# JINXER000/GIE-mapping

Measured on AMD Instinct MI355X. Metric: edt_map_update_throughput, higher is better.
Workload: dtype int32; 1 GPU; 512x512x512 @ 0.05 m, sensor-less hash world (BASELINE config 5): occupied iff hash(x,y,z) < 1 %, full observation, 25 ~; preset=c5, fast_mode=False, tiles=single volume, blocks=360448

## Files before the change

gie-mapping_amd/csrc/gie_api.inc.h:

```cpp
#include <stdio.h>
#include <stdlib.h>
#include <string.h>
#include <math.h>
#include <string>
#include <vector>

#include <cstdio>
#include <unistd.h>
static const char *const gie_kernel_names[GIE_K_NUM] = { "ogm_classify", "ray_register", "ray_free", "ray_finalize", "block_alloc", "fuse",
       "edt_pass_y", "edt_pass_x", "edt_pass_z", "mark", "frontiers", "wave_a", "wave_b", "waves", "commit", "edt_prep", "mark_commit",
       "ground_frontier", "ground_nf1", "ground", "ground_query", "cloud", "los", "los_query", "sdf", "sdf_query" };

#define GIE_REHASH_PERIOD 64
static thread_local std::string g_gie_err;
static void gie_set_err(const std::string &s) { g_gie_err = s; }
extern "C" const char *gie_last_error(void) { return g_gie_err.c_str(); }

enum gie_owed {
    GIE_OWED_NONE,
    GIE_OWED_FRESH,
    GIE_OWED_STALE
};
struct gie_pivots { int pvt[3], upvt[3], tb0[3]; };
struct gie_pair_state {
// ... 1237 lines not shown
    const int n = (face < 0 || face > 5) ? -1 : gie_face_count(m->c, face);
    if (n < 0 || count < 0 || count > n || (count > 0 && !in)) { gie_set_err("gie_halo_import_sparse: bad arguments"); return GIE_ERR_INVALID; }
    if (count == 0) return GIE_OK;
    char *d = (char *)gie_scratch(m, 1, (size_t)count * sizeof(gie_halo_entry) + 16, "gie_halo_import_sparse");
    if (!d) return GIE_ERR_DEVICE;
    be_h2d(&m->be, d, &count, sizeof(int32_t));
    be_h2d(&m->be, d + 16, in, (size_t)count * sizeof(gie_halo_entry));
    rc = gie_halo_import_sparse_dev(m, face, (const gie_halo_entry *)(d + 16), (const int32_t *)d);
    be_sync(&m->be);
    return rc;
}
static int gie_face_set_of(const gie_ctx &c, const void *const p[6], gie_face_set *fs)
{
    int n = 0;
    for (int f = 0; f < 6; f++) { fs->off[f] = n; if (p[f]) n += gie_face_count(c, f); }
    fs->off[6] = n;
    return n;
}
extern "C" int gie_halo_export_all_dev(gie_mapper *m, gie_halo_voxel *const d_out[6])
{
    int rc = gie_need_pose(m, "gie_halo_export_all"); if (rc) return rc;
    if (!d_out) { gie_set_err("gie_halo_export_all: bad arguments"); return GIE_ERR_INVALID; }
    gie_table_for_pose(m);
    op_halo_export_all op;
    const int n = gie_face_set_of(m->c, (const void *const *)d_out, &op.fs);
    for (int f = 0; f < 6; f++) op.out[f] = d_out[f];
    be_lin(&m->be, m->c, op, n);
    return GIE_OK;
}
extern "C" int gie_halo_import_all_dev(gie_mapper *m, const gie_halo_voxel *const d_in[6])
{
    int rc = gie_need_pose(m, "gie_halo_import_all"); if (rc) return rc;
    if (!d_in) { gie_set_err("gie_halo_import_all: bad arguments"); return GIE_ERR_INVALID; }
    op_halo_need_all nd; op_halo_import_all im;
    const int n = gie_face_set_of(m->c, (const void *const *)d_in, &nd.fs);
    im.fs = nd.fs;
    for (int f = 0; f < 6; f++) { nd.in[f] = d_in[f]; im.in[f] = d_in[f]; }
    if (n == 0) return GIE_OK;
    be_lin(&m->be, m->c, nd, n);
    gie_ghost_block_alloc(m);
    be_lin(&m->be, m->c, im, n);
    return GIE_OK;
}
extern "C" int gie_refine(gie_mapper *m, int32_t *seeded)
{
    int rc = gie_need_pose(m, "gie_refine"); if (rc) return rc;
    gie_table_for_pose(m);
    gie_ctx &c = m->c;
    {
        gie_clear_list l; l.n = 0;
        l.p[l.n] = c.cnt + GIE_CNT_C; l.bytes[l.n++] = sizeof(int32_t);
        l.p[l.n] = c.cnt + GIE_CNT_BAR_B; l.bytes[l.n++] = 2 * sizeof(int32_t);
        l.p[l.n] = c.lvl_next; l.bytes[l.n++] = 2 * GIE_MAX_LEVELS * sizeof(int32_t);
        be_clear(&m->be, l, c.gate);
    }
    const int nb = 2 * (c.X * c.Y + c.Y * c.Z + c.X * c.Z);
    be_lin(&m->be, c, op_refine(), nb);
    gie_pp_set_fused(m);
    be_waves(&m->be, c, 0, 0, 0);
    if (!c.fused) be_vox_list<true>(&m->be, c, op_commit(), c.tl_known, GIE_CNT_TL_KNOWN, 0);
    if (!seeded) return GIE_OK;
    rc = gie_sync(m);
    *seeded = m->h_cnt[GIE_CNT_FRONT_C];
    return rc;
}
extern "C" int gie_round_gate(gie_mapper *m, const int32_t *d_go)
{
    if (!m) { gie_set_err("gie_round_gate: null handle"); return GIE_ERR_INVALID; }
    m->c.gate = d_go;
    return GIE_OK;
}
extern "C" int gie_refine_dev(gie_mapper *m, int32_t *d_changed)
{
    if (!d_changed) { gie_set_err("gie_refine_dev: bad arguments"); return GIE_ERR_INVALID; }
    int rc = gie_refine(m, nullptr); if (rc) return rc;
    be_round_note(&m->be, m->c, d_changed, m->d_round_stats, nullptr, 0);
    return GIE_OK;
}
extern "C" int gie_round_end(gie_mapper *m, const int32_t *d_go)
{
    if (!m) { gie_set_err("gie_round_end: null handle"); return GIE_ERR_INVALID; }
    m->c.gate = nullptr;
    be_round_note(&m->be, m->c, nullptr, m->d_round_stats, d_go, 1);
    return GIE_OK;
}
extern "C" int gie_round_stats(gie_mapper *m, int64_t out[4])
{
    if (!m || !out) { gie_set_err("gie_round_stats: bad arguments"); return GIE_ERR_INVALID; }
    long long v[4] = { 0, 0, 0, 0 };
    be_d2h(&m->be, v, m->d_round_stats, sizeof(v));
    for (int i = 0; i < 4; i++) out[i] = (int64_t)v[i];
    return gie_sync(m);
}
extern "C" int gie_get_stream(gie_mapper *m, void **stream)
{
    if (!m || !stream) { gie_set_err("gie_get_stream: bad arguments"); return GIE_ERR_INVALID; }
    *stream = be_stream_handle(&m->be);
    return GIE_OK;
}

#if defined(GIE_TEST_HOOKS)
extern "C" int gie_debug_place_probe(gie_mapper *m, int reps, float *ms)
{
    if (!m || !ms || m->has_pose) { gie_set_err("gie_debug_place_probe: only on a fresh mapper"); return GIE_ERR_INVALID; }
    *ms = be_place_probe(&m->be, m->c, reps > 0 ? (reps & 0xffff) : 3, (reps >> 16) ? (reps >> 16) : 15);
    return gie_sync(m);
}
extern "C" int gie_debug_fault_barrier(gie_mapper *m, int updates)
{
    if (!m || updates < 0) { gie_set_err("gie_debug_fault_barrier: bad arguments"); return GIE_ERR_INVALID; }
    m->bar_fault_left = updates;
    return GIE_OK;
}
extern "C" int gie_debug_nbr_check(gie_mapper *m, int32_t *mismatches)
{
    if (!m || !mismatches) { gie_set_err("gie_debug_nbr_check: bad arguments"); return GIE_ERR_INVALID; }
    int32_t *d = (int32_t *)gie_scratch(m, 0, sizeof(int32_t), "gie_debug_nbr_check");
    if (!d) return GIE_ERR_DEVICE;
    be_memset(&m->be, d, 0, sizeof(int32_t));
    op_nbr_check op; op.bad = d;
    be_lin(&m->be, m->c, op, 6 * m->c.max_blocks);
    be_d2h(&m->be, mismatches, d, sizeof(int32_t));
    return gie_sync(m);
}
enum { GIE_DBG_TS_PREV_VALID = 0, GIE_DBG_TS_COC_DEFER, GIE_DBG_TS_LAZY_OK, GIE_DBG_TS_ZSTREAM, GIE_DBG_TS_ZWIDE, GIE_DBG_TS_ZFAIL,
       GIE_DBG_TS_LAZY_EXACT, GIE_DBG_TS_TSKIP, GIE_DBG_TS_STATE1, GIE_DBG_TS_STATE2, GIE_DBG_TS_NUM };
extern "C" int gie_debug_tile_state(gie_mapper *m, uint8_t *tknown, uint8_t *tskip, uint8_t *tlazy, int32_t *tmax, int32_t *tbmax,
                                    uint32_t *zredo, int32_t *scalars)
{
    if (!m || !scalars) { gie_set_err("gie_debug_tile_state: bad arguments"); return GIE_ERR_INVALID; }
    const gie_ctx &c = m->c;
    const size_t ntile = (size_t)c.tfd[0] * c.tfd[1] * c.tfd[2];
    if (be_sync(&m->be) != 0) return GIE_ERR_DEVICE;
    if (tknown) be_d2h(&m->be, tknown, c.tknown, ntile);
    if (tskip) be_d2h(&m->be, tskip, c.tskip, ntile);
    if (tlazy) be_d2h(&m->be, tlazy, c.tlazy, ntile);
    if (tmax) be_d2h(&m->be, tmax, c.tmax, ntile * sizeof(int32_t));
    if (tbmax) be_d2h(&m->be, tbmax, c.tbmax, ntile * sizeof(int32_t));
    if (zredo) be_d2h(&m->be, zredo, c.zredo, (size_t)((c.X + 15) / 16) * c.Y * sizeof(uint32_t));
    int32_t cnt[GIE_CNT_NUM];
    be_d2h(&m->be, cnt, c.cnt, sizeof(cnt));
    scalars[GIE_DBG_TS_PREV_VALID] = m->pp.owed == GIE_OWED_FRESH;
    scalars[GIE_DBG_TS_COC_DEFER] = c.coc_defer;
    scalars[GIE_DBG_TS_LAZY_OK] = c.lazy_ok;
    scalars[GIE_DBG_TS_ZSTREAM] = cnt[GIE_CNT_ZSTREAM];
    scalars[GIE_DBG_TS_ZWIDE] = cnt[GIE_CNT_ZWIDE];
    scalars[GIE_DBG_TS_ZFAIL] = cnt[GIE_CNT_ZFAIL];
    scalars[GIE_DBG_TS_LAZY_EXACT] = cnt[GIE_CNT_LAZY_EXACT];
    scalars[GIE_DBG_TS_TSKIP] = cnt[GIE_CNT_TSKIP];
    scalars[GIE_DBG_TS_STATE1] = cnt[GIE_CNT_STATE1];
    scalars[GIE_DBG_TS_STATE2] = cnt[GIE_CNT_STATE2];
    return be_sync(&m->be) != 0 ? GIE_ERR_DEVICE : GIE_OK;
}
extern "C" int gie_debug_set_frame(gie_mapper *m, int ct)
{
    if (!m || ct < 0) { gie_set_err("gie_debug_set_frame: bad arguments"); return GIE_ERR_INVALID; }
    if (m->merge_open) { gie_set_err("gie_debug_set_frame: a merge is open (gie_merge_end first)"); return GIE_ERR_INVALID; }
    m->c.map_ct = ct;
    return GIE_OK;
}
#endif
extern "C" int gie_profile_enable(gie_mapper *m, int on)
{
    if (!m) { gie_set_err("gie_profile_enable: null handle"); return GIE_ERR_INVALID; }
    be_prof_enable(&m->be, on);
    return GIE_OK;
}
extern "C" int gie_profile_read(gie_mapper *m, gie_kernel_time *out, int max_entries)
{
    if (!m || !out || max_entries < GIE_K_NUM) { gie_set_err("gie_profile_read: need room for all kernels"); return GIE_ERR_INVALID; }
    float ms[GIE_K_NUM]; int n[GIE_K_NUM];
    be_prof_collect(&m->be, ms, n, GIE_K_NUM);
    int k = 0;
    for (int i = 0; i < GIE_K_NUM; i++) {
        if (i == GIE_K_GROUND_FRONTIER && !m->gfr.planes) continue;
        memset(out[k].name, 0, sizeof(out[k].name));
        strncpy(out[k].name, gie_kernel_names[i], sizeof(out[k].name) - 1);
        out[k].total_ms = ms[i]; out[k].launches = n[i];
        k++;
    }
    return k;
}
```

gie-mapping_amd/csrc/gie_hip.hip:

```cpp
#include <cstdio>
#include <unistd.h>
#include <cstring>
#include <cstdlib>
#include <string>
#include <algorithm>
#include <vector>
#include <hip/hip_runtime.h>
#include <hip/hip_ext.h>
#include <rocprim/rocprim.hpp>
#include "gie_kernels.hip.h"

#define GIE_NEV 8

struct be_state {
    int device;
    int num_cu;
    int cu_total;
    hipStream_t stream;
    hipEvent_t ev[GIE_NEV];
    int ev_set[GIE_NEV];
    void *scan_tmp; size_t scan_bytes;
    void *arena;
    hipEvent_t copy_ev[2];
    hipStream_t side;
// ... 281 lines not shown
    const size_t tile = ((size_t)c.Z * (TX + 1) + 3) & ~(size_t)3;
    const size_t lds = tile * 4 + (size_t)WAVES * LP * 8 + (size_t)LP * 2 + 16;
    static bool attr_done = false;
    if (!attr_done) {
        GIE_HIP_OK(hipFuncSetAttribute(reinterpret_cast<const void *>(&k_edt_z<CP, TX, WAVES>), hipFuncAttributeMaxDynamicSharedMemorySize, 160 * 1024));
        attr_done = true;
    }
    const int ntx = (c.X + TX - 1) / TX, ntiles = ntx * c.Y;
    int wgs = (int)((160 * 1024) / (lds + 256));
    if (wgs < 1) wgs = 1; if (wgs > 4) wgs = 4;
    int grid = wgs * b->cu_total; if (grid > (ntiles + 1) / 2) grid = (ntiles + 1) / 2;
    GIE_LAUNCH(b, (k_edt_z<CP, TX, WAVES>), dim3(grid), dim3(64 * WAVES), lds, c, ntx, ntiles, full);
}
template <int CP> static void gie_launch_edt_xz(be_state *b, const gie_ctx &c, bool zpass, int full, int zs_fused = 0, bool redo = false)
{
    if (redo) {
        GIE_LAUNCH(b, k_edt_x_redo<CP>, dim3(b->cu_total * 8), dim3(64 * GIE_EDTX_WAVES), 0, c);
    } else if (!zpass) {
        GIE_LAUNCH(b, k_edt_x<CP>, dim3((c.Y + GIE_EDTX_WAVES - 1) / GIE_EDTX_WAVES, c.Z), dim3(64 * GIE_EDTX_WAVES), 0, c, zs_fused, full);
    } else {
        gie_launch_edt_z<CP, 16, 8>(b, c, full);
    }
}
static void gie_launch_edt_dim(be_state *b, const gie_ctx &c, int L, bool zpass, int full, int zs_fused = 0, bool redo = false)
{
    if (L <= 64) gie_launch_edt_xz<1>(b, c, zpass, full, zs_fused, redo);
    else if (L <= 128) gie_launch_edt_xz<2>(b, c, zpass, full, zs_fused, redo);
    else if (L <= 256) gie_launch_edt_xz<4>(b, c, zpass, full, zs_fused, redo);
    else if (L <= 512) gie_launch_edt_xz<8>(b, c, zpass, full, zs_fused, redo);
    else gie_launch_edt_xz<16>(b, c, zpass, full, zs_fused, redo);
}
static int be_zs_mode(const gie_ctx &c)
{
    if (c.Z < 64 || c.Z > 1024) return 0;
    static const int fused = GIE_SWITCH("GIE_ZS_FUSED", 1);
    return (fused && (c.X & 1) == 0) ? 2 : 1;
}
static int be_edt_z_stream(be_state *b, const gie_ctx &c, int full);
static void be_edt_z_rest(be_state *b, const gie_ctx &c, int full, int zs)
{
    if (zs == 2) gie_launch_edt_dim(b, c, c.X, false, full, 0, true);
    gie_launch_edt_dim(b, c, c.Z, true, full);
}
static void be_edt_z(be_state *b, const gie_ctx &c, int full) { be_edt_z_rest(b, c, full, be_edt_z_stream(b, c, full) ? be_zs_mode(c) : 0); }
#define GIE_VOXA_MULT 32
template <bool STAGED, class F> static void be_vox_list(be_state *b, const gie_ctx &c, const F &f, const int32_t *list, int count_idx, int always_list)
{
    GIE_LAUNCH(b, (k_voxa<F, STAGED>), dim3(b->cu_total * GIE_VOXA_MULT), dim3(256), 0, c, f, list, count_idx, always_list);
}
#define GIE_MARKC_MULT 64
#define GIE_MARKC_LAZY_MULT 40
static void be_markc(be_state *b, const gie_ctx &c, const int32_t *list)
{
    const dim3 g(b->cu_total * ((c.coc_defer && c.lazy_ok) ? GIE_MARKC_LAZY_MULT : GIE_MARKC_MULT)), t(256);
    GIE_LAUNCH(b, k_markc, g, t, 0, c, list);
}
static float be_place_probe(be_state *b, const gie_ctx &c, int reps, int streams = 15)
{
    const long long ntile = (long long)c.tfd[0] * c.tfd[1] * c.tfd[2];
    const int nslot = (int)(ntile < c.max_blocks ? ntile : c.max_blocks);
    hipEvent_t e0, e1;
    if (hipEventCreate(&e0) != hipSuccess || hipEventCreate(&e1) != hipSuccess) return -1.f;
    std::vector<float> ms;
    hipLaunchKernelGGL(k_place_probe, dim3(b->cu_total * GIE_MARKC_MULT), dim3(256), 0, b->stream, c, nslot, streams);
    for (int r = 0; r < reps; r++) {
        (void)hipEventRecord(e0, b->stream);
        hipLaunchKernelGGL(k_place_probe, dim3(b->cu_total * GIE_MARKC_MULT), dim3(256), 0, b->stream, c, nslot, streams);
        (void)hipEventRecord(e1, b->stream);
        (void)hipEventSynchronize(e1);
        float t = 0.f; (void)hipEventElapsedTime(&t, e0, e1); ms.push_back(t);
    }
    (void)hipEventDestroy(e0); (void)hipEventDestroy(e1);
    std::sort(ms.begin(), ms.end());
    GIE_HIP_OK(hipMemsetAsync(c.pair, 0, (size_t)c.N * sizeof(uint64_t), b->stream));
    return ms.empty() ? -1.f : ms[ms.size() / 2];
}
#define GIE_ROWS_MULT 32
static void be_fuse(be_state *b, const gie_ctx &c, const int32_t *list)
{
    if (c.pntcld_mode) GIE_LAUNCH(b, k_fuse_rows<true>, dim3(b->cu_total * GIE_ROWS_MULT), dim3(256), 0, c, op_fuse(), list);
    else GIE_LAUNCH(b, k_fuse_rows<false>, dim3(b->cu_total * GIE_ROWS_MULT), dim3(256), 0, c, op_fuse(), list);
}
static void be_frontier_tiles(be_state *b, const gie_ctx &c, const int32_t *known, int known_idx, const int32_t *list, int count_idx)
{
    gie_face_patches fp;
    const int da[6] = { c.Y, c.Y, c.X, c.X, c.X, c.X }, db[6] = { c.Z, c.Z, c.Z, c.Z, c.Y, c.Y };
    fp.off[0] = 0;
    for (int f = 0; f < 6; f++) { fp.na[f] = (da[f] + 7) / 8; fp.off[f + 1] = fp.off[f] + fp.na[f] * ((db[f] + 7) / 8); }
    const long long ntile = (long long)c.tfd[0] * c.tfd[1] * c.tfd[2];
    int nsum = (int)((ntile + 64 * GIE_FF_WAVES - 1) / (64 * GIE_FF_WAVES));
    if (nsum > 2 * b->cu_total) nsum = 2 * b->cu_total;
    const int nface = (fp.off[6] + GIE_FF_WAVES - 1) / GIE_FF_WAVES;
    GIE_LAUNCH(b, k_frontier_faces, dim3(nsum + nface), dim3(64 * GIE_FF_WAVES), 0, c, fp, known, known_idx, nsum);
    static int mult = 0;
    if (mult <= 0) {
        if (hipOccupancyMaxActiveBlocksPerMultiprocessor(&mult, reinterpret_cast<const void *>(&k_frontier_tiles), 64 * GIE_FR_WAVES, 0) != hipSuccess || mult < 1) mult = 2;
    }
    GIE_LAUNCH(b, k_frontier_tiles, dim3(b->cu_total * mult), dim3(64 * GIE_FR_WAVES), 0, c, list, count_idx);
}
static void be_edt_z_direct(be_state *b, const gie_ctx &c)
{
    GIE_LAUNCH(b, k_edt_z_direct, dim3(b->cu_total * 16), dim3(256), 0, c);
}
#define GIE_ZSTREAM_WAVES 8
static int be_edt_z_stream(be_state *b, const gie_ctx &c, int full)
{
    const int zs = be_zs_mode(c);
    if (!zs) return 0;
    const int nxr = (c.X + 63) / 64;
    const long long want = (long long)b->cu_total * 4 * GIE_ZSTREAM_WAVES;
    int nseg = (int)((want + (long long)nxr * c.Y - 1) / ((long long)nxr * c.Y));
    const int maxseg = c.Z / 64 > 0 ? c.Z / 64 : 1;
    if (nseg > maxseg) nseg = maxseg; if (nseg < 1) nseg = 1;
    int seg_len = ((c.Z + nseg - 1) / nseg + 31) & ~31;
    nseg = (c.Z + seg_len - 1) / seg_len;
    const long long waves = (long long)nxr * nseg * c.Y;
    long long grid = (waves + 3) / 4;
    const long long cap = (long long)b->cu_total * 8 * 4;
    if (grid > cap) grid = cap;
    if (!full && grid < (long long)b->cu_total * 16) grid = (long long)b->cu_total * 16;
    if (zs == 2) GIE_LAUNCH(b, k_edt_z_stream<true>, dim3((unsigned)grid), dim3(256), 0, c, full, nseg, seg_len, zs);
    else GIE_LAUNCH(b, k_edt_z_stream<false>, dim3((unsigned)grid), dim3(256), 0, c, full, nseg, seg_len, zs);
    return 1;
}
static void be_tile_oldskip(be_state *b, const gie_ctx &c, const int pupvt[3])
{
    const int ntile = c.tfd[0] * c.tfd[1] * c.tfd[2];
    int32_t *const count = &c.cnt[GIE_CNT_STATE1];
    GIE_LAUNCH(b, k_tile_oldskip, dim3((ntile + 255) / 256), dim3(256), 0, c, ntile, c.wc_list[0], count);
    if (c.catchup_fast) GIE_LAUNCH(b, k_coc_catchup_new, dim3(b->cu_total * 8), dim3(256), 0, c, pupvt[0], pupvt[1], pupvt[2], c.wc_list[0], count);
}
static void be_pair_materialise(be_state *b, const gie_ctx &c, int stay)
{
    const int ntile = c.tfd[0] * c.tfd[1] * c.tfd[2];
    int32_t *const count = &c.cnt[GIE_CNT_STATE2];
    GIE_LAUNCH(b, k_pair_lazy_list, dim3((ntile + 255) / 256), dim3(256), 0, c, ntile, stay, c.wc_list[1], count);
    GIE_LAUNCH(b, k_pair_lazy_run, dim3(b->cu_total * 8), dim3(256), 0, c, c.wc_list[1], count);
}
static void be_coc_catchup(be_state *b, const gie_ctx &c, const gie_catchup &p)
{
    const int ntile = c.tfd[0] * c.tfd[1] * c.tfd[2];
    int32_t *const count = &c.cnt[GIE_CNT_STATE1];
    GIE_HIP_OK(hipMemsetAsync(count, 0, sizeof(int32_t), b->stream));
    GIE_LAUNCH(b, k_coc_catchup_list, dim3((ntile + 255) / 256), dim3(256), 0, c, p, ntile, c.wc_list[0], count);
    GIE_LAUNCH(b, k_coc_catchup_run, dim3(b->cu_total * 4), dim3(256), 0, c, p, c.wc_list[0], count);
}
static void be_edt_prep(be_state *b, const gie_ctx &c)
{
    const int ncol = c.tfd[0] * c.tfd[1];
    GIE_LAUNCH(b, k_edt_prep, dim3((ncol + GIE_PREP_WAVES - 1) / GIE_PREP_WAVES), dim3(64 * GIE_PREP_WAVES), 0, c, ncol);
}
static void be_edt(be_state *b, const gie_ctx &c, int full)
{
    dim3 gy((c.X + GIE_EDTY_COLS - 1) / GIE_EDTY_COLS, c.Z);
    be_prof(b, GIE_K_EDT_Y, 0);
    if ((c.X & 3) == 0) {
        const int yb = c.Y > 512 ? 32 : 16, nq = (c.Y + yb - 1) / yb;
        dim3 g4((c.X / 4 + GIE_EDTY4_LANES - 1) / GIE_EDTY4_LANES, c.Z), b4(GIE_EDTY4_LANES, nq);
        if (yb == 16) GIE_LAUNCH(b, k_edt_y4<16>, g4, b4, 0, c);
        else GIE_LAUNCH(b, k_edt_y4<32>, g4, b4, 0, c);
    }
    else if (c.Y <= 256) GIE_LAUNCH(b, (k_edt_y<8, 8>), gy, dim3(GIE_EDTY_COLS, 8), 0, c);
    else if (c.Y <= 512) GIE_LAUNCH(b, (k_edt_y<16, 16>), gy, dim3(GIE_EDTY_COLS, 16), 0, c);
    else GIE_LAUNCH(b, (k_edt_y<32, 16>), gy, dim3(GIE_EDTY_COLS, 16), 0, c);
    be_prof(b, GIE_K_EDT_Y, 1);
    const int zs = be_zs_mode(c);
    be_prof(b, GIE_K_EDT_X, 0); gie_launch_edt_dim(b, c, c.X, false, full, zs == 2 ? zs : 0); be_prof(b, GIE_K_EDT_X, 1);
    be_prof(b, GIE_K_EDT_Z, 0);
    const int zl = be_edt_z_stream(b, c, full);
    if (!zl && !full) be_edt_z_direct(b, c);
    be_edt_z_rest(b, c, full, zl ? zs : 0);
    be_prof(b, GIE_K_EDT_Z, 1);
}
template <class F> static void be_chained(be_state *b, const F &enqueue)
{
    std::lock_guard<std::mutex> lock(g_waves_mutex);
    const int dv = b->device & 63;
    (void)hipSetDevice(b->device);
    const bool chain = g_live_mappers[dv] > 1;
    if (chain) {
        if (g_waves_event_set[dv]) GIE_HIP_OK(hipStreamWaitEvent(b->stream, g_waves_event[dv], 0));
        else { GIE_HIP_OK(hipEventCreateWithFlags(&g_waves_event[dv], hipEventDisableTiming)); g_waves_event_set[dv] = true; }
    }
    enqueue();
    if (chain) GIE_HIP_OK(hipEventRecord(g_waves_event[dv], b->stream));
}
static void be_waves(be_state *b, const gie_ctx &c, int with_ab, int record_seeds, int clear_first)
{
    be_chained(b, [&]() {
        if (clear_first) {
            GIE_HIP_OK(hipMemsetAsync(&c.cnt[GIE_CNT_BAR_B], 0, 2 * sizeof(int32_t), b->stream));
            GIE_HIP_OK(hipMemsetAsync(c.lvl_next, 0, 2 * GIE_MAX_LEVELS * sizeof(int32_t), b->stream));
        }
        if (with_ab) GIE_LAUNCH(b, k_waves_ab, dim3(b->num_cu), dim3(GIE_WAVE_THREADS), 0, c);
        GIE_LAUNCH(b, k_waves_c, dim3(b->num_cu), dim3(GIE_WAVE_THREADS), 0, c, with_ab, record_seeds);
    });
}

#include "gie_api.inc.h"
#include "gie_sdf.inc.h"
#include "gie_nf1.inc.h"
#include "gie_costmat.inc.h"
#include "gie_frontier.inc.h"
#include "gie_los.inc.h"
#include "gie_path.inc.h"
#include "gie_cloud.inc.h"
#include "gie_ground.inc.h"
#include "gie_ground_nf1.inc.h"
#include "gie_ground_los.inc.h"
#include "gie_ground_frontier.inc.h"
#include "gie_ground_costmat.inc.h"
#include "gie_ground_view.inc.h"
#include "gie_ground_rollout.inc.h"
#include "gie_ground_footprint.inc.h"
#include "gie_ground_pose_nf1.inc.h"
```

gie-mapping_amd/csrc/gie_kernels.hip.h:

```cpp
#ifndef GIE_KERNELS_HIP_H
#define GIE_KERNELS_HIP_H

#include <hip/hip_runtime.h>
#include "gie_functors.h"

#if defined(GIE_WAVE_TIMING) || defined(GIE_RAY_TIMING)
#include "../../tools/measure/gie_timing.h"
#endif
#if !defined(GIE_WAVE_TIMING)
#define GIE_TS2(tag, n) do { } while (0)
#define GIE_WPROF_DECL do { } while (0)
#define GIE_WPROF_MARK(base) do { } while (0)
#define GIE_WPROF_ADD(i, v) do { } while (0)
#define GIE_WPROF_END(base) do { } while (0)
#define GIE_WPROF_DRAIN() do { } while (0)
#define GIE_WPROF_SUB(i) do { } while (0)
#define GIE_WPROF_SUBSTART() do { } while (0)
#define GIE_WPROF_DUMP() do { } while (0)
#define GIE_WPROF_CLK() 0ull
#define GIE_WAVE_TIMING_RESET(cond) do { } while (0)
#endif
#if !defined(GIE_RAY_TIMING)
#define GIE_RTS(k) do { } while (0)
#endif
// ... 179 lines not shown
    if (walk) {
        int stop = 0x7fffffff;
        bool more = true;
        for (int k0 = 0; k0 < max_steps && more && stop == 0x7fffffff; k0 += GIE_RAY_BATCH) {
            if (*(volatile int *)&s_stop[lane] < base) break;
            int ids[GIE_RAY_BATCH], end[GIE_RAY_BATCH];
            bool went[GIE_RAY_BATCH];
#pragma unroll
            for (int j = 0; j < GIE_RAY_BATCH; j++) {
                went[j] = gie_dda_before(d, Tn);
                end[j] = 0; ids[j] = -1;
                if (went[j]) { int lx, ly, lz; end[j] = gie_dda_step(d); ids[j] = gie_ray_cell(c, d, lx, ly, lz); }
            }
            int8_t ty[GIE_RAY_BATCH];
#pragma unroll
            for (int j = 0; j < GIE_RAY_BATCH; j++) ty[j] = ids[j] >= 0 ? c.inst_type[ids[j]] : (int8_t)GIE_VOX_UNKNOWN;
#pragma unroll
            for (int j = 0; j < GIE_RAY_BATCH; j++) {
                if (stop != 0x7fffffff || !went[j]) continue;
                if (ty[j] == GIE_VOX_OCCUPIED) stop = base + k0 + j;
                else if (end[j]) stop = base + k0 + j + 1;
            }
            more = went[GIE_RAY_BATCH - 1];
        }
        if (stop != 0x7fffffff) atomicMin(&s_stop[lane], stop);
    }
    GIE_RTS(2);
    __syncthreads();
    GIE_RTS(3);
    const int stop = s_stop[lane];
    d = at_start;
    for (int k = 0; k < max_steps; k++) {
        int id = -1;
        const bool went = walk && base + k < stop && gie_dda_before(d, Tn);
        if (went) {
            int lx, ly, lz;
            gie_dda_step(d);
            id = gie_ray_cell(c, d, lx, ly, lz);
            if (id >= 0) gie_ray_touch_k(c, d, lx, ly, lz, &last_tile);
        }
        if (__ballot(went) == 0ull) break;
        if (__ballot(id >= 0) == 0ull) continue;
        gie_wave_add(c, id, -1);
    }
    GIE_RTS(4);
}

__device__ __forceinline__ void gie_clear_part(const gie_clear_list &l, int w)
{
    int r = 0, nw = gie_clear_wgs(l.bytes[0]);
    while (w >= nw && r + 1 < l.n) { w -= nw; r++; nw = gie_clear_wgs(l.bytes[r]); }
    if (w >= nw) return;
    unsigned char *p = (unsigned char *)l.p[r];
    const uint32_t bytes = l.bytes[r];
    const uint32_t head = (uint32_t)((16u - ((uintptr_t)p & 15u)) & 15u) < bytes ? (uint32_t)((16u - ((uintptr_t)p & 15u)) & 15u) : bytes;
    const uint32_t nvec = (bytes - head) / 16u, tail0 = head + nvec * 16u;
    const uint32_t tid = (uint32_t)w * 256u + threadIdx.x, nth = (uint32_t)nw * 256u;
    for (uint32_t i = tid; i < head; i += nth) p[i] = 0;
    uint4 *v = (uint4 *)(p + head);
    for (uint32_t i = tid; i < nvec; i += nth) v[i] = make_uint4(0, 0, 0, 0);
    for (uint32_t i = tail0 + tid; i < bytes; i += nth) p[i] = 0;
}
__global__ __launch_bounds__(256) void k_clear(const gie_clear_list l, const int32_t *gate)
{
    if (gate != nullptr && *(const volatile int32_t *)gate == 0) return;
    gie_clear_part(l, (int)blockIdx.x);
}

__global__ __launch_bounds__(256) void k_flush_clear(const gie_ctx c, const op_pair_flush f, const int n, const gie_clear_list l, const int nclr)
{
    if ((int)blockIdx.x >= nclr) { const int i = ((int)blockIdx.x - nclr) * 256 + (int)threadIdx.x; if (i < n) f(c, i); return; }
    gie_clear_part(l, (int)blockIdx.x);
}

__global__ __launch_bounds__(256) void k_cell_alloc(const gie_ctx c, const int ncell)
{
    if (GIE_GATE_CLOSED(c)) return;
    const int i = blockIdx.x * 256 + threadIdx.x;
    int found = -1;
    bool isnew = false;
    if (i < ncell) {
        const int bx = i % c.tdim[0], by = (i / c.tdim[0]) % c.tdim[1], bz = i / (c.tdim[0] * c.tdim[1]);
        found = gie_cell_prev_slot(c, bx, by, bz);
        if (found < 0) found = gie_hash_find(c, bx + c.tb0[0], by + c.tb0[1], bz + c.tb0[2]);
        isnew = found < 0 && (c.blk_need[i] || (c.scan_labels && gie_block_observed(c, c.scan_labels, bx, by, bz)));
        c.blk_need[i] = 0;
    }
    __shared__ int s_cnt[4], s_base[4];
    const int lane = __lane_id(), wave = threadIdx.x >> 6;
    const unsigned long long m = __ballot(isnew);
    if (lane == 0) s_cnt[wave] = __popcll(m);
    __syncthreads();
    const int c0 = s_cnt[0], c1 = s_cnt[1], c2 = s_cnt[2], c3 = s_cnt[3];
    const int cnt = c0 + c1 + c2 + c3;
    if (cnt > 0) {
        if (threadIdx.x == 0) {
            int ftop = 0, nf = 0, base = 0;
            if (c.retain > 0) { ftop = atomicSub(&c.pool_count[1], cnt); nf = ftop < 0 ? 0 : (ftop < cnt ? ftop : cnt); }
            if (cnt > nf) base = atomicAdd(&c.pool_count[0], cnt - nf);
            const int lbase = atomicAdd(&c.cnt[GIE_CNT_NEWLIST], cnt);
            atomicAdd(&c.cnt[GIE_CNT_NEWBLK], cnt);
            s_base[0] = base; s_base[1] = lbase; s_base[2] = nf; s_base[3] = ftop;
        }
        __syncthreads();
        if (isnew) {
            const int base = s_base[0], lbase = s_base[1], nf = s_base[2], ftop = s_base[3];
            const int before = (wave > 0 ? c0 : 0) + (wave > 1 ? c1 : 0) + (wave > 2 ? c2 : 0);
            const int r = before + __popcll(m & ((1ull << lane) - 1ull));
            const int slot = gie_alloc_slot(c, r, nf, ftop, base);
            if (slot >= c.max_blocks) { gie_aor32(&c.cnt[GIE_CNT_ERR], GIE_ERRF_POOL); c.blk_new[lbase + r] = -1; }
            else { gie_cell_insert(c, i, slot); c.blk_new[lbase + r] = slot; found = slot; }
        }
    }
    if (i < ncell) {
        c.blk_tab[i] = found;
        if (found >= 0) gie_cell_mark_tiles(c, i);
    }
}
__global__ __launch_bounds__(256) void k_block_init_list(const gie_ctx c, const int ninit, const int ntile)
{
    if (GIE_GATE_CLOSED(c)) return;
    if ((int)blockIdx.x >= ninit) {
        const op_fuse_list f;
        const int nfl = (int)gridDim.x - ninit;
        for (int i0 = ((int)blockIdx.x - ninit) * 256; i0 < ntile; i0 += nfl * 256) {
            const int i = i0 + (int)threadIdx.x;
            f(c, i < ntile ? i : -1);
        }
        return;
    }
    const int n = c.cnt[GIE_CNT_NEWLIST];
    if (blockIdx.x == 0 && threadIdx.x == 0) {
        if (c.pool_count[0] > c.max_blocks) c.pool_count[0] = c.max_blocks;
        if (c.pool_count[1] < 0) c.pool_count[1] = 0;
    }
    for (int e = blockIdx.x; e < n; e += ninit) {
        const int slot = c.blk_new[e];
        if (slot < 0) continue;
        gie_init_voxel(c, slot, threadIdx.x);
        gie_init_voxel(c, slot, threadIdx.x + 256);
        if (threadIdx.x < 6) gie_nbr_link(c, slot, (int)threadIdx.x);
    }
}

#ifndef GIE_EDTY_COLS
#define GIE_EDTY_COLS 64
#endif
template <int YW, int TPC>
__global__ __launch_bounds__(GIE_EDTY_COLS * TPC) void k_edt_y(const gie_ctx c)
{
    constexpr int QW = YW / TPC;
    __shared__ uint32_t s_bits[YW][GIE_EDTY_COLS];
    const int col = threadIdx.x, q = threadIdx.y;
    const int x = blockIdx.x * GIE_EDTY_COLS + col;
    const int z = blockIdx.y;
    if (!c.zocc[z]) return;
    const int X = c.X, Y = c.Y;
    const bool in = x < X;
    const int8_t *t = c.glb_type + (size_t)z * X * Y + (in ? x : 0);
#pragma unroll
    for (int j = 0; j < QW; j++) {
        const int w = q * QW + j;
        uint32_t m = 0;
        if (in && w * 32 < Y) {
#pragma unroll
            for (int k = 0; k < 32; k++) {
                const int y = w * 32 + k;
                if (y < Y) m |= (uint32_t)(t[(size_t)y * X] == GIE_VOX_OCCUPIED) << k;
            }
        }
        s_bits[w][col] = m;
    }
    __syncthreads();
    if (!in) return;
    uint32_t bits[YW];
#pragma unroll
    for (int w = 0; w < YW; w++) bits[w] = s_bits[w][col];
    int prev_last[YW], next_first[YW];
    int last = -1;
#pragma unroll
    for (int w = 0; w < YW; w++) { prev_last[w] = last; if (bits[w]) last = w * 32 + 31 - __clz(bits[w]); }
    int first = -1;
#pragma unroll
    for (int w = YW - 1; w >= 0; w--) { next_first[w] = first; if (bits[w]) first = w * 32 + __ffs(bits[w]) - 1; }
    uint16_t *out = c.cy1 + (size_t)z * X * Y + x;
#pragma unroll
    for (int w = 0; w < YW; w++) {
        if (w / QW != q) continue;
        if (w * 32 >= Y) break;
        const uint32_t bw = bits[w];
        const int pl = prev_last[w], nf = next_first[w];
        for (int k = 0; k < 32; k++) {
            const int y = w * 32 + k;
            if (y >= Y) break;
            const uint32_t lo = bw & (0xffffffffu >> (31 - k));
            const int below = lo ? w * 32 + 31 - __clz(lo) : pl;
            const uint32_t hi = bw >> k;
            const int above = hi ? y + __ffs(hi) - 1 : nf;
            int r;
            if (above >= 0 && (below < 0 || above - y <= y - below)) r = above; else r = below;
            out[(size_t)y * X] = r < 0 ? (uint16_t)0xffff : (uint16_t)r;
        }
    }
}

#define GIE_EDTY4_LANES 16
template <int YB>
__global__ __launch_bounds__(32 * GIE_EDTY4_LANES) void k_edt_y4(const gie_ctx c)
{
    __shared__ __attribute__((aligned(16))) uint32_t s_m[32][GIE_EDTY4_LANES * 4];
    const int l = threadIdx.x, q = threadIdx.y, nq = blockDim.y;
    const int x = (blockIdx.x * GIE_EDTY4_LANES + l) * 4;
    const int z = blockIdx.y;
    if (!c.zocc[z]) return;
    const int X = c.X, Y = c.Y;
    const bool in = x < X;
    const size_t base = (size_t)z * X * Y + (in ? x : 0);
    uint32_t m[4] = {0u, 0u, 0u, 0u};
    if (in) {
        const int8_t *t = c.glb_type + base;
        uint32_t v[YB];
#pragma unroll
        for (int k = 0; k < YB; k++) {
            const int y = q * YB + k;
            v[k] = *reinterpret_cast<const uint32_t *>(t + (size_t)min(y, Y - 1) * X);
        }
        const uint32_t ymask = (q * YB + YB <= Y) ? 0xffffffffu : ((q * YB < Y) ? (0xffffffffu >> (32 - (Y - q * YB))) : 0u);
#pragma unroll
        for (int k = 0; k < YB; k++) {
#pragma unroll
            for (int cc = 0; cc < 4; cc++) m[cc] |= (uint32_t)(((v[k] >> (8 * cc)) & 0xffu) == (uint32_t)GIE_VOX_OCCUPIED) << k;
        }
#pragma unroll
        for (int cc = 0; cc < 4; cc++) m[cc] &= ymask;
    }
    *reinterpret_cast<uint4 *>(&s_m[q][4 * l]) = make_uint4(m[0], m[1], m[2], m[3]);
    __syncthreads();
    if (!in) return;
    int pl[4] = {-1, -1, -1, -1}, nf[4] = {-1, -1, -1, -1};
    for (int w = 0; w < q; w++) {
        const uint4 o = *reinterpret_cast<const uint4 *>(&s_m[w][4 * l]);
        const uint32_t ow[4] = {o.x, o.y, o.z, o.w};
#pragma unroll
        for (int cc = 0; cc < 4; cc++) if (ow[cc]) pl[cc] = w * YB + 31 - __clz(ow[cc]);
    }
    for (int w = nq - 1; w > q; w--) {
        const uint4 o = *reinterpret_cast<const uint4 *>(&s_m[w][4 * l]);
        const uint32_t ow[4] = {o.x, o.y, o.z, o.w};
#pragma unroll
        for (int cc = 0; cc < 4; cc++) if (ow[cc]) nf[cc] = w * YB + __ffs(ow[cc]) - 1;
    }
    uint16_t *out = c.cy1 + base;
#pragma unroll
    for (int k = 0; k < YB; k++) {
        const int y = q * YB + k;
        if (y >= Y) break;
        uint32_t r4[4];
#pragma unroll
        for (int cc = 0; cc < 4; cc++) {
            const uint32_t bw = m[cc];
            const uint32_t lo = bw & (0xffffffffu >> (31 - k));
            const int below = lo ? q * YB + 31 - __clz(lo) : pl[cc];
            const uint32_t hi = bw >> k;
            const int above = hi ? y + __ffs(hi) - 1 : nf[cc];
            int r;
            if (above >= 0 && (below < 0 || above - y <= y - below)) r = above; else r = below;
            r4[cc] = r < 0 ? 0xffffu : (uint32_t)r;
        }
        *reinterpret_cast<uint2 *>(out + (size_t)y * X) = make_uint2(r4[0] | (r4[1] << 16), r4[2] | (r4[3] << 16));
    }
}

__device__ __forceinline__ void gie_wave_sync()
{
    __builtin_amdgcn_fence(__ATOMIC_RELEASE, "wavefront");
    __builtin_amdgcn_wave_barrier();
    __builtin_amdgcn_fence(__ATOMIC_ACQUIRE, "wavefront");
}

__device__ __forceinline__ uint32_t gie_scan_sites(const uint2 *ce, const int up, const int lo, const int hi)
{
    uint32_t b0 = 0xffffffffu, b1 = 0xffffffffu, b2 = 0xffffffffu, b3 = 0xffffffffu;
    for (int j = lo; j <= hi; j += 4) {
        const uint2 v0 = ce[j], v1 = ce[min(j + 1, hi)], v2 = ce[min(j + 2, hi)], v3 = ce[min(j + 3, hi)];
        const int d0 = up - (int)(v0.y & 0xffffu), d1 = up - (int)(v1.y & 0xffffu);
        const int d2 = up - (int)(v2.y & 0xffffu), d3 = up - (int)(v3.y & 0xffffu);
        b0 = min(b0, (uint32_t)__mul24(d0, d0) + v0.x);
        b1 = min(b1, (uint32_t)__mul24(d1, d1) + v1.x);
        b2 = min(b2, (uint32_t)__mul24(d2, d2) + v2.x);
        b3 = min(b3, (uint32_t)__mul24(d3, d3) + v3.x);
    }
    return min(min(b0, b1), min(b2, b3));
}

template <int CP>
__device__ __forceinline__ void gie_row_argmin(const uint2 *ce, const int K, const int L, const int lane, int (&sj)[CP])
{
    const int u0 = lane * CP;
    int s0;
    {
        const int g8 = lane & ~7, r = lane & 7;
        const int ug = g8 * CP;
        uint32_t b0 = 0xffffffffu, b1 = 0xffffffffu, b2 = 0xffffffffu, b3 = 0xffffffffu;
        {
            const int up = ug << 5, kl = K - 1;
            for (int j = r; j < K; j += 32) {
                const uint2 v0 = ce[j], v1 = ce[min(j + 8, kl)], v2 = ce[min(j + 16, kl)], v3 = ce[min(j + 24, kl)];
                const int d0 = up - (int)(v0.y & 0xffffu), d1 = up - (int)(v1.y & 0xffffu);
                const int d2 = up - (int)(v2.y & 0xffffu), d3 = up - (int)(v3.y & 0xffffu);
                b0 = min(b0, (uint32_t)__mul24(d0, d0) + v0.x);
                b1 = min(b1, (uint32_t)__mul24(d1, d1) + v1.x);
                b2 = min(b2, (uint32_t)__mul24(d2, d2) + v2.x);
                b3 = min(b3, (uint32_t)__mul24(d3, d3) + v3.x);
            }
        }
        uint32_t bg = min(min(b0, b1), min(b2, b3));
        bg = min(bg, (uint32_t)__shfl_xor((int)bg, 1));
        bg = min(bg, (uint32_t)__shfl_xor((int)bg, 2));
        bg = min(bg, (uint32_t)__shfl_xor((int)bg, 4));
        const int sg = (ug < L) ? (int)(bg & 1023u) : K - 1;
        int sn = __shfl_down(sg, 8);
        if (lane >= 56) sn = K - 1;
        s0 = sg;
        if (r != 0 && u0 < L && sn > sg) s0 = (int)(gie_scan_sites(ce, u0 << 5, sg, sn) & 1023u);
        if (u0 >= L) s0 = K - 1;
    }
    int sup = __shfl_down(s0, 1);
    if (lane == 63) sup = K - 1;
    int sx[CP + 1];
    sx[0] = s0; sx[CP] = sup;
#pragma unroll
    for (int step = CP / 2; step >= 1; step >>= 1) {
#pragma unroll
        for (int m = step; m < CP; m += 2 * step) {
            const int u = u0 + m;
            const int lo = sx[m - step], hi = sx[m + step];
            int r = lo;
            if (u < L && hi > lo) r = (int)(gie_scan_sites(ce, u << 5, lo, hi) & 1023u);
            sx[m] = (u < L) ? r : K - 1;
        }
    }
#pragma unroll
    for (int m = 0; m < CP; m++) sj[m] = sx[m];
}

#define GIE_BAND_MAXK 160
template <int CP>
__device__ __forceinline__ void gie_row_argmin_banded(const uint2 *ce, const int K, const int L, const int lane, int (&sj)[CP], const unsigned bandneed = ~0u)
{
    constexpr int G = 64 / CP;
    const int b = lane / G, r = lane % G;
    uint32_t b0 = 0xffffffffu, b1 = 0xffffffffu;
    {
        const int up = (64 * b) << 5, kl = K - 1;
        for (int j = r; j < K; j += 2 * G) {
            const uint2 v0 = ce[j], v1 = ce[min(j + G, kl)];
            const int d0 = up - (int)(v0.y & 0xffffu), d1 = up - (int)(v1.y & 0xffffu);
            b0 = min(b0, (uint32_t)__mul24(d0, d0) + v0.x);
            b1 = min(b1, (uint32_t)__mul24(d1, d1) + v1.x);
        }
    }
    uint32_t bg = min(b0, b1);
#pragma unroll
    for (int w = 1; w < G; w <<= 1) bg = min(bg, (uint32_t)__shfl_xor((int)bg, w));
    const int sg = (64 * b < L) ? (int)(bg & 1023u) : K - 1;
    int sa[CP + 1];
#pragma unroll
    for (int m = 0; m < CP; m++) sa[m] = __builtin_amdgcn_readlane(sg, m * G);
    sa[CP] = K - 1;
#pragma unroll
    for (int m = 0; m < CP; m++) {
        if (!((bandneed >> m) & 1u)) { sj[m] = 0; continue; }
        const int lo = sa[m], hi = sa[m + 1];
        const int up = (64 * m + lane) << 5;
        uint32_t c0 = 0xffffffffu, c1 = 0xffffffffu, c2 = 0xffffffffu, c3 = 0xffffffffu;
        for (int j = lo; j <= hi; j += 4) {
            const uint2 v0 = ce[j], v1 = ce[min(j + 1, hi)], v2 = ce[min(j + 2, hi)], v3 = ce[min(j + 3, hi)];
            const int d0 = up - (int)(v0.y & 0xffffu), d1 = up - (int)(v1.y & 0xffffu);
            const int d2 = up - (int)(v2.y & 0xffffu), d3 = up - (int)(v3.y & 0xffffu);
            c0 = min(c0, (uint32_t)__mul24(d0, d0) + v0.x);
            c1 = min(c1, (uint32_t)__mul24(d1, d1) + v1.x);
            c2 = min(c2, (uint32_t)__mul24(d2, d2) + v2.x);
            c3 = min(c3, (uint32_t)__mul24(d3, d3) + v3.x);
        }
        sj[m] = (int)(min(min(c0, c1), min(c2, c3)) & 1023u);
    }
}

#ifndef GIE_BAND_TRIP
#define GIE_BAND_TRIP 8
#endif
#define GIE_BAND_PAD 16
__device__ __forceinline__ void gie_row_mb_pad(int2 *mb, const int K, const int lane)
{
    if (lane < GIE_BAND_PAD - 1) mb[K + lane] = make_int2(0, 0x7fffffff);
}
template <int CP>
__device__ __forceinline__ void gie_row_argmin_banded_lin(const int2 *mb, const int K, const int L, const int lane, int (&sj)[CP])
{
    constexpr int G = 64 / CP;
    const int b = lane / G, r = lane % G;
    int b0 = 0x7fffffff, b1 = 0x7fffffff, b2 = 0x7fffffff, b3 = 0x7fffffff;
    {
        const int u = 64 * b, kl = K - 1;
        for (int j = r; j < K; j += 4 * G) {
            const int2 v0 = mb[j], v1 = mb[min(j + G, kl)], v2 = mb[min(j + 2 * G, kl)], v3 = mb[min(j + 3 * G, kl)];
            b0 = min(b0, __mul24(u, v0.x) + v0.y);
            b1 = min(b1, __mul24(u, v1.x) + v1.y);
            b2 = min(b2, __mul24(u, v2.x) + v2.y);
            b3 = min(b3, __mul24(u, v3.x) + v3.y);
        }
    }
    int bg = min(min(b0, b1), min(b2, b3));
#pragma unroll
    for (int w = 1; w < G; w <<= 1) bg = min(bg, __shfl_xor(bg, w));
    const int sg = (64 * b < L) ? (bg & 1023) : K - 1;
    int sa[CP + 1];
#pragma unroll
    for (int m = 0; m < CP; m++) sa[m] = __builtin_amdgcn_readlane(sg, m * G);
    sa[CP] = K - 1;
#pragma unroll
    for (int m = 0; m < CP; m++) {
// ... 2631 lines not shown
```

gie-mapping_amd/csrc/gie_ops.h:

```cpp
#ifndef GIE_OPS_H
#define GIE_OPS_H

#include "gie_types.h"

#ifndef GIE_PLATFORM_DEFINED
#include "gie_platform.h"
#endif

GIE_DEV void gie_push64(const gie_ctx &c, uint64_t *q, int32_t *counter, int cap, uint64_t v)
{
    const int i = gie_aadd32(counter, 1);
    if (i < cap) gie_st(&q[i], v); else gie_aor32(&c.cnt[GIE_CNT_ERR], GIE_ERRF_QUEUE);
}
GIE_DEV void gie_push64a(const gie_ctx &c, uint64_t *q, gie_vaddr *qaddr, int32_t *counter, int cap, uint64_t v, gie_vaddr a)
{
    const int i = gie_aadd32(counter, 1);
    if (i < cap) { gie_st(&q[i], v); gie_st(&qaddr[i], a); } else gie_aor32(&c.cnt[GIE_CNT_ERR], GIE_ERRF_QUEUE);
}
GIE_DEV void gie_push64a_wave(const gie_ctx &c, uint64_t *q, gie_vaddr *qaddr, int32_t *counter, int cap, bool push, uint64_t v, gie_vaddr a)
{
    const unsigned long long m = __ballot(push);
    if (!m) return;
    const int lane = __lane_id(), leader = __ffsll((long long)m) - 1;
    int base = 0;
// ... 1142 lines not shown
{
    const gie_halo_voxel h = gie_halo_record(c, face, i);
    const bool known = h.vox_type != GIE_VOX_UNKNOWN;
    const unsigned long long m = __ballot(known);
    if (!m) return;
    const int lane = __lane_id(), leader = __ffsll((long long)m) - 1;
    int base = 0;
    if (lane == leader) base = gie_aadd32(count, __popcll(m));
    base = __shfl(base, leader);
    if (known) { const int s = base + __popcll(m & ((1ull << lane) - 1ull)); out[s].index = i; out[s].v = h; }
}
GIE_DEV void gie_halo_need_rec(const gie_ctx &c, int face, int i, const gie_halo_voxel &v)
{
    if (v.vox_type == GIE_VOX_UNKNOWN) return;
    int x, y, z;
    gie_face_coord(c, face, i, 1, &x, &y, &z);
    c.blk_need[gie_tab_index(c, x + c.pvt[0], y + c.pvt[1], z + c.pvt[2])] = 1;
}
GIE_DEV void gie_halo_need_voxel(const gie_ctx &c, int face, int i, const gie_halo_voxel *in) { gie_halo_need_rec(c, face, i, in[i]); }
GIE_DEV void gie_halo_import_rec(const gie_ctx &c, int face, int i, const gie_halo_voxel &v)
{
    if (v.vox_type == GIE_VOX_UNKNOWN) return;
    int x, y, z;
    gie_face_coord(c, face, i, 1, &x, &y, &z);
    const gie_vaddr a = gie_gvox_tab(c, x + c.pvt[0], y + c.pvt[1], z + c.pvt[2]);
    if (a < 0) return;
    c.g_type[a] = v.vox_type;
    c.g_occ[a] = v.occ_val;
    c.g_coc[a] = gie_pack_crd(v.coc[0], v.coc[1], v.coc[2]);
    gie_touch(c, a);
}
GIE_DEV void gie_halo_import_voxel(const gie_ctx &c, int face, int i, const gie_halo_voxel *in) { gie_halo_import_rec(c, face, i, in[i]); }
GIE_DEV void gie_halo_need_entry(const gie_ctx &c, int face, int j, const gie_halo_entry *in, const int32_t *count, int nface)
{
    if (j >= *count) return;
    const gie_halo_entry e = in[j];
    if ((unsigned)e.index < (unsigned)nface) gie_halo_need_rec(c, face, e.index, e.v);
}
GIE_DEV void gie_halo_import_entry(const gie_ctx &c, int face, int j, const gie_halo_entry *in, const int32_t *count, int nface)
{
    if (j >= *count) return;
    const gie_halo_entry e = in[j];
    if ((unsigned)e.index < (unsigned)nface) gie_halo_import_rec(c, face, e.index, e.v);
}
GIE_DEV int gie_refine_voxel(const gie_ctx &c, int id)
{
    const int x = id % c.X, y = (id / c.X) % c.Y, z = id / (c.X * c.Y);
    if (c.glb_type[id] == GIE_VOX_UNKNOWN) return 0;
    const int cd = gie_pair_dist(c.pair[id]);
    uint64_t seed = 0;
    int hit = 0;
    const int dx[6] = { -1, 1, 0, 0, 0, 0 }, dy[6] = { 0, 0, -1, 1, 0, 0 }, dz[6] = { 0, 0, 0, 0, -1, 1 };
    GIE_UNROLL6
    for (int k = 0; k < 6; k++) {
        const int nx = x + dx[k], ny = y + dy[k], nz = z + dz[k];
        if (gie_in_loc(c, nx, ny, nz)) continue;
        const gie_vaddr a = gie_gvox_tab(c, nx + c.pvt[0], ny + c.pvt[1], nz + c.pvt[2]);
        if (a < 0 || c.g_type[a] == GIE_VOX_UNKNOWN) continue;
        if (gie_invalid_dist(c, gie_gdist(c, c.g_coc[a], nx + c.pvt[0], ny + c.pvt[1], nz + c.pvt[2]))) continue;
        int ncx, ncy, ncz;
        gie_unpack_crd(c.g_coc[a], &ncx, &ncy, &ncz);
        if (gie_invalid_coc(ncx, ncy, ncz)) continue;
        const int nw[3] = { ncx - c.upvt[0], ncy - c.upvt[1], ncz - c.upvt[2] };
        const int nl[3] = { ncx - c.pvt[0], ncy - c.pvt[1], ncz - c.pvt[2] };
        const int hidden = gie_in_whole(c, nx, ny, nz) ? !gie_in_loc(c, nl[0], nl[1], nl[2]) : !gie_in_whole(c, nl[0], nl[1], nl[2]);
        if (!hidden || !gie_in_wr(c, nw[0], nw[1], nw[2])) continue;
        const int d = gie_d2(nl[0], nl[1], nl[2], x, y, z);
        if (d < cd) { seed = gie_pair_make(d, gie_pack_wr(nw[0], nw[1], nw[2])); hit = 1; }
    }
    if (hit) c.cand[1][id] = seed;
    return hit;
}
GIE_DEV int gie_refine_entry(const gie_ctx &c, int j)
{
    int face = 0, i = j;
    for (; face < 6; face++) { const int n = gie_face_count(c, face); if (i < n) break; i -= n; }
    if (face >= 6) return -1;
    int x, y, z;
    gie_face_coord(c, face, i, 0, &x, &y, &z);
    if (face >= 1 && x == 0) return -1;
    if (face >= 2 && x == c.X - 1) return -1;
    if (face >= 3 && y == 0) return -1;
    if (face >= 4 && y == c.Y - 1) return -1;
    if (face >= 5 && z == 0) return -1;
    return gie_lid(c, x, y, z);
}

GIE_DEV void gie_export_pair(const gie_ctx &c, int id, int32_t *dist_sq, int32_t *coc_xyz)
{
    const uint64_t pr = gie_pair_get_id(c, id);
    const int d = gie_pair_dist(pr);
    if (dist_sq) dist_sq[id] = d;
    if (coc_xyz) {
        if (gie_pair_par(pr) == GIE_PAR_NONE || d >= c.empty_value) {
            coc_xyz[3 * id] = coc_xyz[3 * id + 1] = coc_xyz[3 * id + 2] = GIE_EMPTY_VALUE;
        } else {
            int w[3];
            gie_unpack_wr(gie_pair_par(pr), &w[0], &w[1], &w[2]);
            coc_xyz[3 * id] = w[0] + c.upvt[0]; coc_xyz[3 * id + 1] = w[1] + c.upvt[1]; coc_xyz[3 * id + 2] = w[2] + c.upvt[2];
        }
    }
}
GIE_DEV void gie_export_bcoc(const gie_ctx &c, int id, int32_t *dist_sq, int32_t *coc_xyz)
{
    const uint32_t bc = c.bcoc[id];
    if (dist_sq) dist_sq[id] = gie_bcoc_dist(bc, id % c.X, (id / c.X) % c.Y, id / (c.X * c.Y), c.max_width * c.max_width);
    if (!coc_xyz) return;
    if (bc == GIE_BCOC_NONE) { coc_xyz[3 * id] = coc_xyz[3 * id + 1] = coc_xyz[3 * id + 2] = -1; }
    else { coc_xyz[3 * id] = (int)(bc & 1023u); coc_xyz[3 * id + 1] = (int)((bc >> 10) & 1023u); coc_xyz[3 * id + 2] = (int)(bc >> 20); }
}
GIE_DEV void gie_stream_list(const gie_ctx &c, const int32_t *rank, int32_t *list, int slot)
{ if (c.g_dirty[slot]) list[rank[slot]] = slot; }
GIE_DEV void gie_stream_gather(const gie_ctx &c, const int32_t *list, int first, int32_t *keys, gie_voxel *out, int i)
{
    const int slot = list[first + (i >> 9)], j = i & 511;
    const gie_vaddr a = (gie_vaddr)slot * GIE_VBSZ + ((j >> 6) | (((j >> 3) & 7) << 3) | ((j & 7) << 6));
    gie_voxel v;
    v.occ_val = c.g_occ[a]; v.vox_type = c.g_type[a]; v.pad = 0;
    {
        int k[3];
        gie_unpack_crd(c.g_key[slot], &k[0], &k[1], &k[2]);
        const int ib = (int)(a & (GIE_VBSZ - 1));
        v.dist_sq = gie_gdist(c, c.g_coc[a], k[0] * 8 + (ib & 7), k[1] * 8 + ((ib >> 3) & 7), k[2] * 8 + (ib >> 6));
    }
    gie_unpack_crd(c.g_coc[a], &v.coc[0], &v.coc[1], &v.coc[2]);
    out[i] = v;
    if (j < 3) {
        int k[3];
        gie_unpack_crd(c.g_key[slot], &k[0], &k[1], &k[2]);
        keys[3 * (i >> 9) + j] = k[j];
    }
}
GIE_DEV void gie_stream_clear(const gie_ctx &c, const int32_t *list, int first, int i) { c.g_dirty[list[first + i]] = 0; }

GIE_DEV void gie_query_voxel(const gie_ctx &c, const int32_t *xyz, int i, gie_voxel *out)
{
    const gie_vaddr a = gie_gvox_hash(c, xyz[3 * i], xyz[3 * i + 1], xyz[3 * i + 2]);
    out[i].pad = 0;
    uint64_t dcc;
    if (a >= 0 && gie_deferred_coc(c, xyz[3 * i], xyz[3 * i + 1], xyz[3 * i + 2], &dcc)) {
        out[i].occ_val = c.g_occ[a]; out[i].vox_type = c.g_type[a]; out[i].dist_sq = gie_gdist(c, dcc, xyz[3 * i], xyz[3 * i + 1], xyz[3 * i + 2]);
        gie_unpack_crd(dcc, &out[i].coc[0], &out[i].coc[1], &out[i].coc[2]);
        return;
    }
    if (a < 0) {
        out[i].occ_val = 0; out[i].vox_type = GIE_VOX_UNKNOWN; out[i].dist_sq = c.empty_value;
        out[i].coc[0] = out[i].coc[1] = out[i].coc[2] = GIE_EMPTY_VALUE;
    } else {
        out[i].occ_val = c.g_occ[a]; out[i].vox_type = c.g_type[a]; out[i].dist_sq = gie_gdist(c, c.g_coc[a], xyz[3 * i], xyz[3 * i + 1], xyz[3 * i + 2]);
        gie_unpack_crd(c.g_coc[a], &out[i].coc[0], &out[i].coc[1], &out[i].coc[2]);
    }
}

#endif
```

Baseline: 101,000 Mvoxels/s.

## Remap EDT-Y block grid and use SWAR occupancy bits with nonzero-word summary

```diff
diff --git a/gie-mapping_amd/csrc/gie_api.inc.h b/gie-mapping_amd/csrc/gie_api.inc.h
--- a/gie-mapping_amd/csrc/gie_api.inc.h
+++ b/gie-mapping_amd/csrc/gie_api.inc.h
@@ -1413,6 +1413,13 @@
     scalars[GIE_DBG_TS_STATE2] = cnt[GIE_CNT_STATE2];
     return be_sync(&m->be) != 0 ? GIE_ERR_DEVICE : GIE_OK;
 }
+extern "C" int gie_debug_plane_flags(gie_mapper *m, uint8_t *flags)
+{
+    if (!m || !flags) { gie_set_err("gie_debug_plane_flags: bad arguments"); return GIE_ERR_INVALID; }
+    if (be_sync(&m->be) != 0) return GIE_ERR_DEVICE;
+    be_d2h(&m->be, flags, m->c.zocc, (size_t)m->c.Z);
+    return be_sync(&m->be) != 0 ? GIE_ERR_DEVICE : GIE_OK;
+}
 extern "C" int gie_debug_set_frame(gie_mapper *m, int ct)
 {
     if (!m || ct < 0) { gie_set_err("gie_debug_set_frame: bad arguments"); return GIE_ERR_INVALID; }
diff --git a/gie-mapping_amd/csrc/gie_hip.hip b/gie-mapping_amd/csrc/gie_hip.hip
--- a/gie-mapping_amd/csrc/gie_hip.hip
+++ b/gie-mapping_amd/csrc/gie_hip.hip
@@ -457,11 +457,11 @@
 }
 static void be_edt(be_state *b, const gie_ctx &c, int full)
 {
-    dim3 gy((c.X + GIE_EDTY_COLS - 1) / GIE_EDTY_COLS, c.Z);
+    dim3 gy(16 * gie_edty_groups((c.X + GIE_EDTY_COLS - 1) / GIE_EDTY_COLS, c.Z));
     be_prof(b, GIE_K_EDT_Y, 0);
     if ((c.X & 3) == 0) {
         const int yb = c.Y > 512 ? 32 : 16, nq = (c.Y + yb - 1) / yb;
-        dim3 g4((c.X / 4 + GIE_EDTY4_LANES - 1) / GIE_EDTY4_LANES, c.Z), b4(GIE_EDTY4_LANES, nq);
+        dim3 g4(16 * gie_edty_groups((c.X / 4 + GIE_EDTY4_LANES - 1) / GIE_EDTY4_LANES, c.Z)), b4(GIE_EDTY4_LANES, nq);
         if (yb == 16) GIE_LAUNCH(b, k_edt_y4<16>, g4, b4, 0, c);
         else GIE_LAUNCH(b, k_edt_y4<32>, g4, b4, 0, c);
     }
diff --git a/gie-mapping_amd/csrc/gie_kernels.hip.h b/gie-mapping_amd/csrc/gie_kernels.hip.h
--- a/gie-mapping_amd/csrc/gie_kernels.hip.h
+++ b/gie-mapping_amd/csrc/gie_kernels.hip.h
@@ -355,10 +355,11 @@
     constexpr int QW = YW / TPC;
     __shared__ uint32_t s_bits[YW][GIE_EDTY_COLS];
     const int col = threadIdx.x, q = threadIdx.y;
-    const int x = blockIdx.x * GIE_EDTY_COLS + col;
-    const int z = blockIdx.y;
+    const int X = c.X, Y = c.Y;
+    int strip, z;
+    if (!gie_edty_strip(blockIdx.x, (X + GIE_EDTY_COLS - 1) / GIE_EDTY_COLS, c.Z, &strip, &z)) return;
+    const int x = strip * GIE_EDTY_COLS + col;
     if (!c.zocc[z]) return;
-    const int X = c.X, Y = c.Y;
     const bool in = x < X;
     const int8_t *t = c.glb_type + (size_t)z * X * Y + (in ? x : 0);
 #pragma unroll
@@ -412,11 +413,15 @@
 __global__ __launch_bounds__(32 * GIE_EDTY4_LANES) void k_edt_y4(const gie_ctx c)
 {
     __shared__ __attribute__((aligned(16))) uint32_t s_m[32][GIE_EDTY4_LANES * 4];
-    const int l = threadIdx.x, q = threadIdx.y, nq = blockDim.y;
-    const int x = (blockIdx.x * GIE_EDTY4_LANES + l) * 4;
-    const int z = blockIdx.y;
+    __shared__ __attribute__((aligned(16))) uint32_t s_nz[GIE_EDTY4_LANES * 4];
+    const int l = threadIdx.x, q = threadIdx.y;
+    const int X = c.X, Y = c.Y;
+    int strip, z;
+    if (!gie_edty_strip(blockIdx.x, (X / 4 + GIE_EDTY4_LANES - 1) / GIE_EDTY4_LANES, c.Z, &strip, &z)) return;
+    const int x = (strip * GIE_EDTY4_LANES + l) * 4;
     if (!c.zocc[z]) return;
-    const int X = c.X, Y = c.Y;
+    if (q == 0) *reinterpret_cast<uint4 *>(&s_nz[4 * l]) = make_uint4(0u, 0u, 0u, 0u);
+    __syncthreads();
     const bool in = x < X;
     const size_t base = (size_t)z * X * Y + (in ? x : 0);
     uint32_t m[4] = {0u, 0u, 0u, 0u};
@@ -429,48 +434,51 @@
             v[k] = *reinterpret_cast<const uint32_t *>(t + (size_t)min(y, Y - 1) * X);
         }
         const uint32_t ymask = (q * YB + YB <= Y) ? 0xffffffffu : ((q * YB < Y) ? (0xffffffffu >> (32 - (Y - q * YB))) : 0u);
+        uint32_t acc[YB / 8];
+#pragma unroll
+        for (int j = 0; j < YB / 8; j++) acc[j] = 0u;
 #pragma unroll
         for (int k = 0; k < YB; k++) {
-#pragma unroll
-            for (int cc = 0; cc < 4; cc++) m[cc] |= (uint32_t)(((v[k] >> (8 * cc)) & 0xffu) == (uint32_t)GIE_VOX_OCCUPIED) << k;
-        }
-#pragma unroll
-        for (int cc = 0; cc < 4; cc++) m[cc] &= ymask;
+            const uint32_t t2 = v[k] ^ (0x01010101u * (uint32_t)GIE_VOX_OCCUPIED);
+            const uint32_t zb = ~(((t2 & 0x7f7f7f7fu) + 0x7f7f7f7fu) | t2) & 0x80808080u;
+            acc[k >> 3] |= (zb >> 7) << (k & 7);
+        }
+#pragma unroll
+        for (int cc = 0; cc < 4; cc++) {
+#pragma unroll
+            for (int j = 0; j < YB / 8; j++) m[cc] |= ((acc[j] >> (8 * cc)) & 0xffu) << (8 * j);
+            m[cc] &= ymask;
+            if (m[cc]) atomicOr(&s_nz[4 * l + cc], 1u << q);
+        }
     }
     *reinterpret_cast<uint4 *>(&s_m[q][4 * l]) = make_uint4(m[0], m[1], m[2], m[3]);
     __syncthreads();
     if (!in) return;
-    int pl[4] = {-1, -1, -1, -1}, nf[4] = {-1, -1, -1, -1};
-    for (int w = 0; w < q; w++) {
-        const uint4 o = *reinterpret_cast<const uint4 *>(&s_m[w][4 * l]);
-        const uint32_t ow[4] = {o.x, o.y, o.z, o.w};
-#pragma unroll
-        for (int cc = 0; cc < 4; cc++) if (ow[cc]) pl[cc] = w * YB + 31 - __clz(ow[cc]);
-    }
-    for (int w = nq - 1; w > q; w--) {
-        const uint4 o = *reinterpret_cast<const uint4 *>(&s_m[w][4 * l]);
-        const uint32_t ow[4] = {o.x, o.y, o.z, o.w};
-#pragma unroll
-        for (int cc = 0; cc < 4; cc++) if (ow[cc]) nf[cc] = w * YB + __ffs(ow[cc]) - 1;
+    const uint4 nzv = *reinterpret_cast<const uint4 *>(&s_nz[4 * l]);
+    const uint32_t nz[4] = {nzv.x, nzv.y, nzv.z, nzv.w};
+    const uint32_t mlow = (1u << q) - 1u, mhigh = ~((2u << q) - 1u);
+    int pl[4], nf[4];
+#pragma unroll
+    for (int cc = 0; cc < 4; cc++) {
+        const uint32_t b = nz[cc] & mlow, a = nz[cc] & mhigh;
+        const int wb = b ? 31 - __clz(b) : 0, wa = a ? __ffs(a) - 1 : 0;
+        const uint32_t ob = s_m[wb][4 * l + cc], oa = s_m[wa][4 * l + cc];
+        pl[cc] = b ? wb * YB + 31 - __clz(ob) : -65536;
+        nf[cc] = a ? wa * YB + __ffs(oa) - 1 : 65535;
     }
     uint16_t *out = c.cy1 + base;
 #pragma unroll
     for (int k = 0; k < YB; k++) {
         const int y = q * YB + k;
-        if (y >= Y) break;
         uint32_t r4[4];
 #pragma unroll
         for (int cc = 0; cc < 4; cc++) {
-            const uint32_t bw = m[cc];
-            const uint32_t lo = bw & (0xffffffffu >> (31 - k));
-            const int below = lo ? q * YB + 31 - __clz(lo) : pl[cc];
-            const uint32_t hi = bw >> k;
+            const uint32_t hi = m[cc] >> k;
+            pl[cc] = (hi & 1u) ? y : pl[cc];
             const int above = hi ? y + __ffs(hi) - 1 : nf[cc];
-            int r;
-            if (above >= 0 && (below < 0 || above - y <= y - below)) r = above; else r = below;
-            r4[cc] = r < 0 ? 0xffffu : (uint32_t)r;
-        }
-        *reinterpret_cast<uint2 *>(out + (size_t)y * X) = make_uint2(r4[0] | (r4[1] << 16), r4[2] | (r4[3] << 16));
+            r4[cc] = (uint32_t)((above - y <= y - pl[cc]) ? above : pl[cc]);
+        }
+        if (y < Y) *reinterpret_cast<uint2 *>(out + (size_t)y * X) = make_uint2(r4[0] | (r4[1] << 16), r4[2] | (r4[3] << 16));
     }
 }
 
diff --git a/gie-mapping_amd/csrc/gie_ops.h b/gie-mapping_amd/csrc/gie_ops.h
--- a/gie-mapping_amd/csrc/gie_ops.h
+++ b/gie-mapping_amd/csrc/gie_ops.h
@@ -1318,4 +1318,14 @@
     }
 }
 
+GIE_HD int gie_edty_groups(int nstrip, int Z) { return (((nstrip + 1) >> 1) * Z + 7) >> 3; }
+GIE_HD int gie_edty_strip(int l, int nstrip, int Z, int *strip, int *z)
+{
+    const int np = (nstrip + 1) >> 1;
+    const int pair = ((l >> 4) << 3) | (l & 7);
+    *z = pair / np;
+    *strip = 2 * (pair - *z * np) + ((l >> 3) & 1);
+    return *z < Z && *strip < nstrip;
+}
+
 #endif
```

Result: faster. 102,900 Mvoxels/s (median of 6 runs) (+1.9%).
